# tgp-team/torch-geometric-pool

Measured on AMD Instinct MI355X. Metric: pooled nodes/sec (Reduce+Connect) on batched graphs, higher is better.
Workload: dtype f32; 1 GPU; DiffPool dense S^T X / S^T A S, batch=32 graphs N=1024 K=128 F=64 (BASELINE configs[1]); graphs_per_gpu=32, nodes_per_graph=1024, clusters=128, features=64, parallelism=graph-sharded x1

## Files before the change

### torch-geometric-pool_amd/csrc/gemm_mfma.h

```cpp
#pragma once
#include <stdlib.h>
#include <type_traits>

#include "common.h"

namespace tgp {


typedef float f32x16 __attribute__((ext_vector_type(16)));
typedef float f32x4 __attribute__((ext_vector_type(4)));

constexpr int BK = 32;
#ifndef TGP_OPERAND_PREFETCH
#define TGP_OPERAND_PREFETCH 1
#endif
#ifndef TGP_LOAD_AT
#define TGP_LOAD_AT 7
#endif
#ifndef TGP_STORE_AT
#define TGP_STORE_AT 3
#endif
#ifndef TGP_STEADY_LOOP
#define TGP_STEADY_LOOP 1
#endif
#ifndef TGP_SPREAD
#define TGP_SPREAD 1
#endif
#ifndef TGP_MIRROR_ROWS
#define TGP_MIRROR_ROWS 1
#endif
#ifndef TGP_VEC_EPILOGUE
#define TGP_VEC_EPILOGUE 1
#endif

constexpr int LDA_ROWMAJOR = BK + 1;

#ifndef TGP_SPARSE_CHUNK_GROUPS
#define TGP_SPARSE_CHUNK_GROUPS 224
#endif
#ifndef TGP_DENSE_RUN
#define TGP_DENSE_RUN 2
#endif

struct GemmRhs {
  const float* Bm;
  float* C;
  int Nc;
  long ldb, ldc, sB, sC, sCsplit;
};

struct GemmArgs {
  const float* A;
  long lda, sA;
  int M, Kd;
  GemmRhs rhs[3];
  int tiles_m, tiles_n0, tiles_n;
  int tiles_n1;
  int splits;
  int k_per_split;
  const int64_t* k_ptr;
  const int64_t* m_ptr;
  const float* resid;
  long ldr, sR;
  float* partial;
  int force_bm, force_bn;
  const int64_t* sizes;
  int accumulate;
  float* colsum;
  int colsum_skip_diag;
  int symmetric;
};

__device__ __forceinline__ int tile_row(int t) {
  const int g = t >> 3, r = t & 7;
  return 4 * (g & 7) + (r & 3) + 32 * (r >> 2) + 64 * (g >> 3);
}

#ifdef TGP_GEMM_STAMPS
__device__ unsigned long long* g_gemm_stamps = nullptr;
__device__ int g_gemm_reverse = 0;
#define TGP_STAMP(slot)                                                                        \
  do {                                                                                          \
    if (g_gemm_stamps && threadIdx.x == 0)                                                      \
      g_gemm_stamps[static_cast<long>(blockIdx.x) * 16 + (slot)] = __builtin_amdgcn_s_memrealtime(); \
  } while (0)
#else
#define TGP_STAMP(slot) do {} while (0)
#endif

__device__ __forceinline__ float4 ld4_guarded(const float* p, bool ok) {
  return ok ? *reinterpret_cast<const float4*>(p) : make_float4(0.f, 0.f, 0.f, 0.f);
}

template <bool A_KMAJOR, bool ALIGNED, int BM, int BN, int MODE, int WN = 2>
__global__ __launch_bounds__(BM * 2 * WN) void gemm_f32_mfma_kernel(GemmArgs g) {
  constexpr int THREADS = BM * 2 * WN;
  constexpr int NT = BN / (32 * WN);
  constexpr int B_TILE_FLOATS = MODE == 1 ? BN * LDA_ROWMAJOR : BK * BN;
  constexpr int BN_LANES = BN / 4;
  constexpr int A_TILE_FLOATS = BM * LDA_ROWMAJOR;
  constexpr int STAGE_FLOATS = A_TILE_FLOATS + B_TILE_FLOATS;
  constexpr int A_VECS = BM * BK / 4 / THREADS;
  constexpr int B_VECS = BN * BK / 4 / THREADS;
  constexpr int AK_LANES = BM / 4;
  constexpr bool FOLD = MODE == 4;
  constexpr bool SKIP = MODE == 3 || FOLD;
  static_assert(!FOLD || (BM == 128 && BN == 128 && WN == 4), "MODE 4: one 128 x 128 tile, 16 waves as 4 x 4");
  constexpr int NW = THREADS / 64;
  constexpr int S_ROWS = BM / NW, S_COLS = BN / 64;
  static_assert(!SKIP || (ALIGNED && S_ROWS % 2 == 0 && (S_COLS == 1 || S_COLS == 2) && NW <= 16 && BM * BN <= 2 * STAGE_FLOATS),
                "MODE 3: aligned tiles, two rows per ballot, one or two columns per lane");
  constexpr int LDA_KM = SKIP ? BM + 4 : BM;
  static_assert(BK * LDA_KM <= A_TILE_FLOATS, "k-major A tile exceeds its LDS slot");
  extern __shared__ __attribute__((aligned(16))) float smem[];
  const int tid = threadIdx.x, lane = tid & 63, wave = tid >> 6;
  const int wm = wave / WN, wn = wave % WN;
  TGP_STAMP(0);
#ifdef TGP_GEMM_STAMPS
  if (g_gemm_stamps && threadIdx.x == 0) {
    unsigned hw, xcc;
    asm volatile("s_getreg_b32 %0, hwreg(HW_REG_HW_ID)" : "=s"(hw));
    asm volatile("s_getreg_b32 %0, hwreg(HW_REG_XCC_ID)" : "=s"(xcc));
    g_gemm_stamps[static_cast<long>(blockIdx.x) * 16 + 4] = hw;
    g_gemm_stamps[static_cast<long>(blockIdx.x) * 16 + 5] = xcc;
  }
#endif

  int bid = xcd_remap(blockIdx.x, gridDim.x);
#ifdef TGP_GEMM_STAMPS
  if (g_gemm_reverse) bid = gridDim.x - 1 - bid;
#endif
  const int tn_all = bid % g.tiles_n; bid /= g.tiles_n;
  const int tm = bid % g.tiles_m; bid /= g.tiles_m;
  const int split = bid % g.splits;
  const int batch = bid / g.splits;
  const int which = tn_all >= g.tiles_n0 ? ((g.tiles_n1 && tn_all >= g.tiles_n1) ? 2 : 1) : 0;
  const int tn = which == 2 ? tn_all - g.tiles_n1 : (which ? tn_all - g.tiles_n0 : tn_all);
  const GemmRhs& R = g.rhs[which];

  const float* __restrict__ A = g.A + static_cast<long>(batch) * g.sA;
  const float* __restrict__ Bm = R.Bm + static_cast<long>(batch) * R.sB;
  float* __restrict__ C = R.C + static_cast<long>(batch) * R.sC + static_cast<long>(split) * R.sCsplit;
  const int Nc = R.Nc;
  const long lda = g.lda, ldb = R.ldb;

  const int m0 = tm * BM, n0 = tn * BN;
  if constexpr (MODE == 1) {
    if (g.sizes) {
      const int64_t nb = g.sizes[batch];
      if (m0 >= nb || n0 >= nb) {
        if (threadIdx.x == 0)
          g.partial[static_cast<long>(batch) * (g.tiles_m * g.tiles_n) + tm * g.tiles_n + tn_all] = 0.f;
        return;
      }
    }
    if (g.symmetric && m0 > n0) {
      if (threadIdx.x == 0)
        g.partial[static_cast<long>(batch) * (g.tiles_m * g.tiles_n) + tm * g.tiles_n + tn_all] = 0.f;
      return;
    }
  }
  int M = g.M;
  if (g.m_ptr) {
    const long m_lo = g.m_ptr[batch];
    M = static_cast<int>(g.m_ptr[batch + 1] - m_lo);
    if (m0 >= M) return;
    A += m_lo * lda;
    C += m_lo * R.ldc;
  }
  int k_lo = 0, k_hi = g.Kd;
  if (g.k_ptr) {
    k_lo = static_cast<int>(g.k_ptr[batch]);
    k_hi = static_cast<int>(g.k_ptr[batch + 1]);
  }
  const int k_begin = k_lo + split * g.k_per_split;
  const int k_end = min(k_hi, k_begin + g.k_per_split);
  const int nk = k_end > k_begin ? (k_end - k_begin + BK - 1) / BK : 0;

  float4 ra[2][A_VECS], rb[2][B_VECS];

  constexpr int OOB = static_cast<int>(0x80000000u);
  [[maybe_unused]] __amdgpu_buffer_rsrc_t rsrc_a, rsrc_b;
  [[maybe_unused]] int voff_a[A_VECS], voff_b[B_VECS];
  [[maybe_unused]] int kloc_a[A_VECS], kloc_b[B_VECS];
  if constexpr (ALIGNED) {
    const int a_bytes = A_KMAJOR ? (static_cast<int>(g.Kd - 1) * static_cast<int>(lda) + M) * 4
                                 : (static_cast<int>(M - 1) * static_cast<int>(lda) + g.Kd) * 4;
    const int b_bytes = MODE == 1 ? (static_cast<int>(Nc - 1) * static_cast<int>(ldb) + g.Kd) * 4
                                  : (static_cast<int>(g.Kd - 1) * static_cast<int>(ldb) + Nc) * 4;
    rsrc_a = __builtin_amdgcn_make_buffer_rsrc(const_cast<float*>(A), 0, a_bytes, 0x00020000);
    rsrc_b = __builtin_amdgcn_make_buffer_rsrc(const_cast<float*>(Bm), 0, b_bytes, 0x00020000);
#pragma unroll
    for (int i = 0; i < A_VECS; ++i) {
      if constexpr (!A_KMAJOR) {
        const int m = m0 + tile_row((tid >> 3) + i * (THREADS / 8));
        kloc_a[i] = (tid & 7) * 4;
        voff_a[i] = m < M ? (m * static_cast<int>(lda) + kloc_a[i]) * 4 : OOB;
      } else {
        const int m = m0 + (tid % AK_LANES) * 4;
        kloc_a[i] = tid / AK_LANES + i * (THREADS / AK_LANES);
        voff_a[i] = m < M ? (kloc_a[i] * static_cast<int>(lda) + m) * 4 : OOB;
      }
    }
#pragma unroll
    for (int i = 0; i < B_VECS; ++i) {
      if constexpr (MODE == 1) {
        const int n = n0 + tile_row((tid >> 3) + i * (THREADS / 8));
        kloc_b[i] = (tid & 7) * 4;
        voff_b[i] = n < Nc ? (n * static_cast<int>(ldb) + kloc_b[i]) * 4 : OOB;
      } else {
        const int n = n0 + (tid % BN_LANES) * 4;
        kloc_b[i] = tid / BN_LANES + i * (THREADS / BN_LANES);
        voff_b[i] = n < Nc ? (kloc_b[i] * static_cast<int>(ldb) + n) * 4 : OOB;
      }
    }
  }
  auto buf_ld4 = [&](__amdgpu_buffer_rsrc_t r, int voff, int soff) {
    typedef unsigned int u32x4 __attribute__((ext_vector_type(4)));
    const u32x4 v = __builtin_amdgcn_raw_buffer_load_b128(r, voff, soff, 0);
    return make_float4(__uint_as_float(v.x), __uint_as_float(v.y), __uint_as_float(v.z), __uint_as_float(v.w));
  };

  auto load_a = [&](int i, int k0, bool tail) -> float4 {
    if constexpr (ALIGNED) {
      const int soff = A_KMAJOR ? k0 * static_cast<int>(lda) * 4 : k0 * 4;
      if (!tail) return buf_ld4(rsrc_a, voff_a[i], soff);
      float4 v = buf_ld4(rsrc_a, k0 + kloc_a[i] < k_end ? voff_a[i] : OOB, soff);
      if constexpr (!A_KMAJOR) {
        const int rem = k_end - (k0 + kloc_a[i]);
        if (rem < 4) { v.w = 0.f; if (rem < 3) v.z = 0.f; if (rem < 2) v.y = 0.f; }
      }
      return v;
    } else {
      int m, k;
      if constexpr (!A_KMAJOR) {
        m = m0 + tile_row((tid >> 3) + i * (THREADS / 8));
        k = k0 + (tid & 7) * 4;
      } else {
        k = k0 + tid / AK_LANES + i * (THREADS / AK_LANES);
        m = m0 + (tid % AK_LANES) * 4;
      }
      const float* p = A_KMAJOR ? A + static_cast<long>(k) * lda + m : A + static_cast<long>(m) * lda + k;
      float t[4];
#pragma unroll
      for (int j = 0; j < 4; ++j) {
        const bool ok = A_KMAJOR ? (k < k_end && m + j < M) : (m < M && k + j < k_end);
        t[j] = ok ? p[j] : 0.f;
      }
      return make_float4(t[0], t[1], t[2], t[3]);
    }
  };
  auto load_b = [&](int i, int k0, bool tail) -> float4 {
    if constexpr (ALIGNED) {
      const int soff = MODE == 1 ? k0 * 4 : k0 * static_cast<int>(ldb) * 4;
      if (!tail) return buf_ld4(rsrc_b, voff_b[i], soff);
      float4 v = buf_ld4(rsrc_b, k0 + kloc_b[i] < k_end ? voff_b[i] : OOB, soff);
      if constexpr (MODE == 1) {
        const int rem = k_end - (k0 + kloc_b[i]);
        if (rem < 4) { v.w = 0.f; if (rem < 3) v.z = 0.f; if (rem < 2) v.y = 0.f; }
      }
      return v;
    } else {
      float t[4];
      if constexpr (MODE == 1) {
        const int n = n0 + tile_row((tid >> 3) + i * (THREADS / 8)), k = k0 + (tid & 7) * 4;
        const float* p = Bm + static_cast<long>(n) * ldb + k;
#pragma unroll
        for (int j = 0; j < 4; ++j) t[j] = (n < Nc && k + j < k_end) ? p[j] : 0.f;
      } else {
        const int k = k0 + tid / BN_LANES + i * (THREADS / BN_LANES), n = n0 + (tid % BN_LANES) * 4;
        const float* p = Bm + static_cast<long>(k) * ldb + n;
#pragma unroll
        for (int j = 0; j < 4; ++j) t[j] = (k < k_end && n + j < Nc) ? p[j] : 0.f;
      }
      return make_float4(t[0], t[1], t[2], t[3]);
    }
  };
  auto store_a = [&](int i, const float4& v, float* As) {
    if constexpr (!A_KMAJOR) {
      float* d = As + tile_row((tid >> 3) + i * (THREADS / 8)) * LDA_ROWMAJOR + (tid & 7) * 4;
      d[0] = v.x; d[1] = v.y; d[2] = v.z; d[3] = v.w;
    } else {
      *reinterpret_cast<float4*>(As + (tid / AK_LANES + i * (THREADS / AK_LANES)) * LDA_KM + (tid % AK_LANES) * 4) = v;
    }
  };
  auto store_b = [&](int i, const float4& v, float* Bs) {
    if constexpr (MODE == 1) {
      float* d = Bs + tile_row((tid >> 3) + i * (THREADS / 8)) * LDA_ROWMAJOR + (tid & 7) * 4;
      d[0] = v.x; d[1] = v.y; d[2] = v.z; d[3] = v.w;
    } else {
      *reinterpret_cast<float4*>(Bs + (tid / BN_LANES + i * (THREADS / BN_LANES)) * BN + (tid % BN_LANES) * 4) = v;
    }
  };

  f32x16 acc[NT];
#pragma unroll
  for (int j = 0; j < NT; ++j)
#pragma unroll
    for (int r = 0; r < 16; ++r) acc[j][r] = 0.f;

  const int lm = lane & 31, lk = lane >> 5;
  float rres[MODE == 1 ? NT : 1][16];
  [[maybe_unused]] float rmir[MODE == 1 ? NT : 1][16];
  [[maybe_unused]] const bool mirror = MODE == 1 && g.symmetric && m0 < n0;
  constexpr bool MIRROR_PATCH_FITS = (THREADS / 64) * (32 * 33) <= 2 * STAGE_FLOATS;
  [[maybe_unused]] const bool mirror_rows = mirror && MIRROR_PATCH_FITS && TGP_MIRROR_ROWS && (g.ldr & 3) == 0 &&
                                            (reinterpret_cast<uintptr_t>(g.resid + static_cast<long>(batch) * g.sR) & 15) == 0 &&
                                            m0 + BM <= M && n0 + BN <= Nc && n0 + BN <= M && m0 + BM <= Nc;
  if constexpr (MODE == 1) {
    const float* __restrict__ Rm = g.resid + static_cast<long>(batch) * g.sR;
#pragma unroll
    for (int j = 0; j < NT; ++j) {
      const int col = n0 + wn * (BN / WN) + j * 32 + lm;
#pragma unroll
      for (int r = 0; r < 16; ++r) {
        const int row = m0 + wm * 32 + (r & 3) + 8 * (r >> 2) + 4 * lk;
        rres[j][r] = (row < M && col < Nc) ? Rm[static_cast<long>(row) * g.ldr + col] : 0.f;
      }
    }
    if (mirror && mirror_rows) {
      const float* __restrict__ base = Rm + static_cast<long>(n0 + wn * (BN / WN) + (lane >> 3)) * g.ldr + m0 + wm * 32 +
                                       4 * (lane & 7);
#pragma unroll
      for (int j = 0; j < NT; ++j)
#pragma unroll
        for (int q = 0; q < 4; ++q) {
          const float4 v = *reinterpret_cast<const float4*>(base + static_cast<long>(j * 32 + 8 * q) * g.ldr);
          rmir[j][4 * q] = v.x; rmir[j][4 * q + 1] = v.y; rmir[j][4 * q + 2] = v.z; rmir[j][4 * q + 3] = v.w;
        }
    } else if (mirror) {
      const bool v4 = (g.ldr & 3) == 0 && (reinterpret_cast<uintptr_t>(Rm) & 15) == 0;
#pragma unroll
      for (int j = 0; j < NT; ++j) {
        const int col = n0 + wn * (BN / WN) + j * 32 + lm;
#pragma unroll
        for (int q = 0; q < 4; ++q) {
          const int row = m0 + wm * 32 + 8 * q + 4 * lk;
          const float* src = Rm + static_cast<long>(col) * g.ldr + row;
          if (v4 && col < Nc && row + 3 < M) {
            const float4 v = *reinterpret_cast<const float4*>(src);
            rmir[j][4 * q] = v.x; rmir[j][4 * q + 1] = v.y; rmir[j][4 * q + 2] = v.z; rmir[j][4 * q + 3] = v.w;
          } else {
#pragma unroll
            for (int u = 0; u < 4; ++u) rmir[j][4 * q + u] = (col < Nc && row + u < M) ? src[u] : 0.f;
          }
        }
      }
    }
  }
  const int a_off = A_KMAJOR ? lk * LDA_KM + wm * 32 + lm : (wm * 32 + lm) * LDA_ROWMAJOR + lk;
  const int a_step = A_KMAJOR ? 2 * LDA_KM : 2;
  const int b_off = MODE == 1 ? (wn * (BN / WN) + lm) * LDA_ROWMAJOR + lk : lk * BN + wn * (BN / WN) + lm;
  constexpr int b_step = MODE == 1 ? 2 : 2 * BN;
  constexpr int b_tile = MODE == 1 ? 32 * LDA_ROWMAJOR : 32;
  constexpr int PD = TGP_OPERAND_PREFETCH;
  float a_r[PD + 1], b_r[PD + 1][NT];
  auto fetch_pair = [&](const float* As, const float* Bs, int p) {
    a_r[p % (PD + 1)] = As[a_off + p * a_step];
#pragma unroll
    for (int j = 0; j < NT; ++j) b_r[p % (PD + 1)][j] = Bs[b_off + p * b_step + b_tile * j];
  };
  auto mfma_pair = [&](int p) {
#pragma unroll
    for (int j = 0; j < NT; ++j)
      acc[j] = __builtin_amdgcn_mfma_f32_32x32x2f32(a_r[p % (PD + 1)], b_r[p % (PD + 1)][j], acc[j], 0, 0, 0);
  };

  [[maybe_unused]] unsigned* chunk_rec = reinterpret_cast<unsigned*>(smem + 2 * STAGE_FLOATS);
  [[maybe_unused]] float sacc[SKIP ? S_ROWS : 1][S_COLS];
  [[maybe_unused]] bool any_sparse = false;
  if constexpr (SKIP) {
#pragma unroll
    for (int j = 0; j < S_ROWS; ++j)
#pragma unroll
      for (int c = 0; c < S_COLS; ++c) sacc[j][c] = 0.f;
  }
  auto record_chunk = [&](auto par, const auto& va, const auto& vb) {
    unsigned n = 0;
#pragma unroll
    for (int i = 0; i < A_VECS; ++i)
      n += __popcll(__ballot(((__float_as_uint(va[i].x) | __float_as_uint(va[i].y) | __float_as_uint(va[i].z) |
                               __float_as_uint(va[i].w)) << 1) != 0u));
    unsigned mag = 0;
#pragma unroll
    for (int i = 0; i < B_VECS; ++i)
      mag = max(max(mag, max(__float_as_uint(vb[i].x) & 0x7fffffffu, __float_as_uint(vb[i].y) & 0x7fffffffu)),
                max(__float_as_uint(vb[i].z) & 0x7fffffffu, __float_as_uint(vb[i].w) & 0x7fffffffu));
    if (__ballot(mag >= 0x7f800000u)) n += 1u << 16;
    if (lane == 0) chunk_rec[par * 16 + wave] = n;
  };
  auto chunk_is_sparse = [&](auto par) -> bool {
    const uint4* r = reinterpret_cast<const uint4*>(chunk_rec + par * 16);
    unsigned n = 0;
#pragma unroll
    for (int q = 0; q < NW / 4; ++q) {
      const uint4 v = r[q];
      n += v.x + v.y + v.z + v.w;
    }
    return __builtin_amdgcn_readfirstlane(n) <= TGP_SPARSE_CHUNK_GROUPS;
  };
  auto sparse_chunk = [&](auto As, auto Bs) {
    float va[S_ROWS / 2];
#pragma unroll
    for (int i = 0; i < S_ROWS / 2; ++i) {
      const int row = wave + NW * (2 * i + (lane >> 5)), k = lane & 31;
      va[i] = A_KMAJOR ? As[k * LDA_KM + row] : As[row * LDA_ROWMAJOR + k];
    }
#pragma unroll
    for (int i = 0; i < S_ROWS / 2; ++i) asm volatile("" : "+v"(va[i]));
#pragma unroll
    for (int i = 0; i < S_ROWS / 2; ++i) {
      const float v = va[i];
      const unsigned long long nz = __ballot(v != 0.f);
      const int vbits = __float_as_int(v);
#pragma unroll
      for (int h = 0; h < 2; ++h) {
        for (unsigned m = static_cast<unsigned>(nz >> (32 * h)); m; m &= m - 1) {
          const int kk = __builtin_ctz(m);
          const float a = __int_as_float(__builtin_amdgcn_readlane(vbits, kk + 32 * h));
          if constexpr (S_COLS == 2) {
            const float2 b = *reinterpret_cast<const float2*>(Bs + kk * BN + 2 * lane);
            sacc[2 * i + h][0] = fmaf(a, b.x, sacc[2 * i + h][0]);
            sacc[2 * i + h][S_COLS - 1] = fmaf(a, b.y, sacc[2 * i + h][S_COLS - 1]);
          } else {
            sacc[2 * i + h][0] = fmaf(a, Bs[kk * BN + lane], sacc[2 * i + h][0]);
          }
        }
      }
    }
  };

  float* L0 = smem;
  float* L1 = smem + STAGE_FLOATS;
  auto kof = [&](int t) { return k_begin + t * BK; };
  [[maybe_unused]] int dense_run = 0;
  [[maybe_unused]] bool dense_rest = false;
  auto stage = [&](auto par_c, auto steady_c, auto sk_c, int t) {
    constexpr int PAR = decltype(par_c)::value;
    constexpr bool STEADY = decltype(steady_c)::value;
    constexpr bool SK = decltype(sk_c)::value;
    const float* As = PAR ? L1 : L0;
    const float* Bs = As + A_TILE_FLOATS;
    float* An = PAR ? L0 : L1;
    float* Bn = An + A_TILE_FLOATS;
    const bool do_store = STEADY || t + 1 < nk, do_load = STEADY || t + 2 < nk;
    const int k2 = kof(t + 2);
    const bool tail = !STEADY && k2 + BK > k_end;
#ifdef TGP_GEMM_STAMPS
    const bool probe = g_gemm_stamps && t == (nk / 2) && threadIdx.x == 0;
#define TGP_PHASE(i) do { if (probe) g_gemm_stamps[static_cast<long>(blockIdx.x) * 16 + 8 + (i)] = __builtin_amdgcn_s_memrealtime(); } while (0)
#else
#define TGP_PHASE(i) do {} while (0)
#endif
    TGP_PHASE(0);
    bool sparse = false;
    if constexpr (SK) {
#pragma unroll
      for (int p = 0; p < PD; ++p) fetch_pair(As, Bs, p);
      sparse = chunk_is_sparse(PAR);
#pragma unroll
      for (int p = 0; p < PD; ++p) {
        asm volatile("" ::"v"(a_r[p % (PD + 1)]));
#pragma unroll
        for (int j = 0; j < NT; ++j) asm volatile("" ::"v"(b_r[p % (PD + 1)][j]));
      }
      any_sparse = any_sparse || sparse;
      dense_run = sparse ? 0 : dense_run + 1;
      dense_rest = dense_run >= TGP_DENSE_RUN;
      if (sparse) {
#pragma unroll
      for (int v = 0; v < A_VECS + B_VECS; ++v)
        if (do_load) {
          if (v < A_VECS) ra[PAR][v] = load_a(v, k2, tail);
          else rb[PAR][v - A_VECS] = load_b(v - A_VECS, k2, tail);
        }
      sparse_chunk(As, Bs);
#pragma unroll
      for (int v = 0; v < A_VECS + B_VECS; ++v)
        if (do_store) {
          if (v < A_VECS) store_a(v, ra[1 - PAR][v], An);
          else store_b(v - A_VECS, rb[1 - PAR][v - A_VECS], Bn);
        }
      if (do_store) record_chunk(1 - PAR, ra[1 - PAR], rb[1 - PAR]);
#pragma unroll
      for (int j = 0; j < NT; ++j) asm volatile("" : "+v"(acc[j]));
      }
    }
    if (!SK || !sparse) {
    if constexpr (!SK) {
#pragma unroll
      for (int p = 0; p < PD; ++p) fetch_pair(As, Bs, p);
    }
#pragma unroll
    for (int p = 0; p < BK / 2; ++p) {
      if (p + PD < BK / 2) fetch_pair(As, Bs, p + PD);
      mfma_pair(p);
      if (p + PD < BK / 2) __builtin_amdgcn_sched_group_barrier(0x100, 1 + NT, 0);
      __builtin_amdgcn_sched_group_barrier(0x008, NT, 0);
      constexpr int LOAD_AT = TGP_LOAD_AT, STORE_AT = TGP_STORE_AT, SPREAD = TGP_SPREAD;
      if (p == STORE_AT) TGP_PHASE(1);
      if (p == LOAD_AT) TGP_PHASE(3);
#pragma unroll
      for (int v = 0; v < A_VECS + B_VECS; ++v) {
        if (p == LOAD_AT + (SPREAD ? v : 0) && do_load) {
          if (v < A_VECS) ra[PAR][v] = load_a(v, k2, tail);
          else rb[PAR][v - A_VECS] = load_b(v - A_VECS, k2, tail);
        }
        if (p == STORE_AT + (SPREAD ? v : 0) && do_store) {
          if (v < A_VECS) store_a(v, ra[1 - PAR][v], An);
          else store_b(v - A_VECS, rb[1 - PAR][v - A_VECS], Bn);
        }
      }
      if constexpr (SK) {
        if (p == STORE_AT + (SPREAD ? A_VECS + B_VECS : 1) && do_store) record_chunk(1 - PAR, ra[1 - PAR], rb[1 - PAR]);
      }
      __builtin_amdgcn_sched_barrier(0);
      if (p == STORE_AT) TGP_PHASE(2);
      if (p == LOAD_AT) TGP_PHASE(4);
    }
    }
    TGP_PHASE(5);
    __syncthreads();
    TGP_PHASE(6);
  };
  if (nk > 0) {
#pragma unroll
    for (int i = 0; i < A_VECS; ++i) ra[0][i] = load_a(i, kof(0), kof(0) + BK > k_end);
#pragma unroll
    for (int i = 0; i < B_VECS; ++i) rb[0][i] = load_b(i, kof(0), kof(0) + BK > k_end);
  }
  if (nk > 1) {
#pragma unroll
    for (int i = 0; i < A_VECS; ++i) ra[1][i] = load_a(i, kof(1), kof(1) + BK > k_end);
#pragma unroll
    for (int i = 0; i < B_VECS; ++i) rb[1][i] = load_b(i, kof(1), kof(1) + BK > k_end);
  }
  if (nk > 0) {
#pragma unroll
    for (int i = 0; i < A_VECS; ++i) store_a(i, ra[0][i], L0);
#pragma unroll
    for (int i = 0; i < B_VECS; ++i) store_b(i, rb[0][i], L0 + A_TILE_FLOATS);
    if constexpr (SKIP) record_chunk(0, ra[0], rb[0]);
  }
  __syncthreads();
  TGP_STAMP(1);
  [[maybe_unused]] float4 fs[4], fx[2];
  auto fold_load = [&]() {
    if constexpr (FOLD) {
      const GemmRhs& RX = g.rhs[1];
      const int x_bytes = RX.Bm ? static_cast<int>(g.Kd) * static_cast<int>(RX.ldb) * 4 : 0;
      const __amdgpu_buffer_rsrc_t rsrc_x = __builtin_amdgcn_make_buffer_rsrc(
          const_cast<float*>(RX.Bm ? RX.Bm + static_cast<long>(batch) * RX.sB : Bm), 0, x_bytes, 0x00020000);
      const int ldx4 = RX.Bm ? static_cast<int>(RX.ldb) * 4 : 0;
      const int voff_x = (RX.Bm && (tid & 15) * 4 < RX.Nc) ? (tid >> 4) * ldx4 + (tid & 15) * 16 : OOB;
#pragma unroll
      for (int i = 0; i < 4; ++i) fs[i] = buf_ld4(rsrc_b, voff_b[0], (m0 + 32 * i) * static_cast<int>(ldb) * 4);
#pragma unroll
      for (int i = 0; i < 2; ++i) fx[i] = buf_ld4(rsrc_x, voff_x, (m0 + 64 * i) * ldx4);
    }
  };
  int t = 0;
  using std::integral_constant;
  using FALSE_C = integral_constant<bool, false>;
  using TRUE_C = integral_constant<bool, true>;
  if constexpr (!SKIP) {
  if constexpr (ALIGNED && TGP_STEADY_LOOP) {
    for (; t + 3 < nk && kof(t + 3) + BK <= k_end; t += 2) {
#ifdef TGP_GEMM_STAMPS
      if (t == (nk / 2 & ~1)) TGP_STAMP(6);
      if (t == ((3 * nk) / 4 & ~1)) TGP_STAMP(7);
#endif
      stage(integral_constant<int, 0>{}, TRUE_C{}, FALSE_C{}, t);
      stage(integral_constant<int, 1>{}, TRUE_C{}, FALSE_C{}, t + 1);
    }
  }
  for (; t < nk; t += 2) {
#ifdef TGP_GEMM_STAMPS
    if (t == (nk / 2 & ~1)) TGP_STAMP(6);
    if (t == ((3 * nk) / 4 & ~1)) TGP_STAMP(7);
#endif
    stage(integral_constant<int, 0>{}, FALSE_C{}, FALSE_C{}, t);
    if (t + 1 < nk) stage(integral_constant<int, 1>{}, FALSE_C{}, FALSE_C{}, t + 1);
  }
  } else {
    for (; t + 3 < nk && kof(t + 3) + BK <= k_end && !dense_rest; t += 2) {
      stage(integral_constant<int, 0>{}, TRUE_C{}, TRUE_C{}, t);
      stage(integral_constant<int, 1>{}, TRUE_C{}, TRUE_C{}, t + 1);
    }
    for (; t + 3 < nk && kof(t + 3) + BK <= k_end; t += 2) {
      stage(integral_constant<int, 0>{}, TRUE_C{}, FALSE_C{}, t);
      stage(integral_constant<int, 1>{}, TRUE_C{}, FALSE_C{}, t + 1);
    }
    auto tail_stage = [&](auto par_c, int t) {
      if (dense_rest) stage(par_c, FALSE_C{}, FALSE_C{}, t);
      else stage(par_c, FALSE_C{}, TRUE_C{}, t);
    };
    for (; t < nk; t += 2) {
      tail_stage(integral_constant<int, 0>{}, t);
      if (t + 1 < nk) tail_stage(integral_constant<int, 1>{}, t + 1);
    }
  }
  TGP_STAMP(2);
  fold_load();
  if constexpr (SKIP && !FOLD) {
    if (any_sparse) {
#pragma unroll
      for (int j = 0; j < S_ROWS; ++j)
#pragma unroll
        for (int c = 0; c < S_COLS; ++c) smem[(wave + NW * j) * BN + S_COLS * lane + c] = sacc[j][c];
      __syncthreads();
#pragma unroll
      for (int j = 0; j < NT; ++j)
#pragma unroll
        for (int r = 0; r < 16; ++r)
          acc[j][r] = __fadd_rn(acc[j][r],
                                smem[(wm * 32 + (r & 3) + 8 * (r >> 2) + 4 * lk) * BN + wn * (BN / WN) + j * 32 + lm]);
      __syncthreads();
    }
  }

  if constexpr (FOLD) {
    constexpr int P_LD = 196;
    float* Sf = smem;
    float* UXf = smem + BM * BN;
    const GemmRhs& RX = g.rhs[1];
    const int F = RX.Bm ? RX.Nc : 0;
    const int l15 = lane & 15, lq = lane >> 4;
#pragma unroll
    for (int i = 0; i < 4; ++i) {
      const int k = (tid >> 5) + 32 * i;
      *reinterpret_cast<float4*>(Sf + k * BN + (((tid & 31) * 4) ^ ((k & 3) << 4))) = fs[i];
    }
#pragma unroll
    for (int i = 0; i < 2; ++i) {
      const int k = (tid >> 4) + 64 * i;
      *reinterpret_cast<float4*>(UXf + k * 192 + ((BN + (tid & 15) * 4) ^ ((k & 3) << 4))) = fx[i];
    }
#pragma unroll
    for (int r = 0; r < 16; ++r) {
      const int rl = (r & 3) + 8 * (r >> 2) + 4 * lk;
      UXf[(wm * 32 + rl) * 192 + ((wn * 32 + lm) ^ ((r & 3) << 4))] = m0 + wm * 32 + rl < M ? acc[0][r] : 0.f;
    }
    f32x4 d[2][3];
#pragma unroll
    for (int i = 0; i < 2; ++i)
#pragma unroll
      for (int j = 0; j < 3; ++j)
#pragma unroll
        for (int r = 0; r < 4; ++r) d[i][j][r] = 0.f;
    __syncthreads();
    if (any_sparse) {
#pragma unroll
      for (int j = 0; j < S_ROWS; ++j) {
        const int row = wave + NW * j;
        float2* u = reinterpret_cast<float2*>(UXf + row * 192 + ((2 * lane) ^ ((row & 3) << 4)));
        float2 v = *u;
        v.x = __fadd_rn(v.x, sacc[j][0]);
        v.y = __fadd_rn(v.y, sacc[j][S_COLS - 1]);
        *u = v;
      }
      __syncthreads();
    }
    TGP_STAMP(8);
    {
      int a_at[2], b_at[3];
#pragma unroll
      for (int i = 0; i < 2; ++i) a_at[i] = lq * BN + ((wm * 32 + 16 * i + l15) ^ (lq << 4));
#pragma unroll
      for (int j = 0; j < 3; ++j) b_at[j] = lq * 192 + ((wn * 48 + 16 * j + l15) ^ (lq << 4));
      float a[2][2], b[2][3];
      auto fetch = [&](int s) {
#pragma unroll
        for (int i = 0; i < 2; ++i) a[s & 1][i] = Sf[4 * s * BN + a_at[i]];
#pragma unroll
        for (int j = 0; j < 3; ++j) b[s & 1][j] = UXf[4 * s * 192 + b_at[j]];
      };
      fetch(0);
#pragma unroll
      for (int s = 0; s < 32; ++s) {
        if (s + 1 < 32) fetch(s + 1);
#pragma unroll
        for (int j = 0; j < 3; ++j)
#pragma unroll
          for (int i = 0; i < 2; ++i)
            d[i][j] = __builtin_amdgcn_mfma_f32_16x16x4f32(a[s & 1][i], b[s & 1][j], d[i][j], 0, 0, 0);
        if (s + 1 < 32) __builtin_amdgcn_sched_group_barrier(0x100, 5, 0);
        __builtin_amdgcn_sched_group_barrier(0x008, 6, 0);
        __builtin_amdgcn_sched_barrier(0);
      }
    }
    TGP_STAMP(9);
    __syncthreads();
    bool used[3];
#pragma unroll
    for (int j = 0; j < 3; ++j) {
      const int c0 = wn * 48 + 16 * j;
      used[j] = c0 < BN ? c0 < Nc : c0 - BN < F;
    }
    float* P = smem;
#pragma unroll
    for (int i = 0; i < 2; ++i)
#pragma unroll
      for (int j = 0; j < 3; ++j)
        if (used[j]) {
#pragma unroll
          for (int r = 0; r < 4; ++r) P[(wm * 32 + 16 * i + 4 * lq + r) * P_LD + wn * 48 + 16 * j + l15] = d[i][j][r];
        }
    __syncthreads();
    TGP_STAMP(10);
    if (g.colsum) {
      float* part = smem + BM * P_LD;
      const int j = tid & (BN - 1), q = tid >> 7;
      float cs = 0.f;
#pragma unroll
      for (int u = 0; u < 16; ++u) {
        const int row = 16 * q + u;
        const float v = P[row * P_LD + j];
        cs = __fadd_rn(cs, (row >= Nc || (g.colsum_skip_diag && row == j)) ? 0.f : v);
      }
      part[q * BN + j] = cs;
      __syncthreads();
      if (tid < Nc) {
        float tot = 0.f;
#pragma unroll
        for (int qq = 0; qq < 8; ++qq) tot = __fadd_rn(tot, part[qq * BN + tid]);
        g.colsum[(static_cast<long>(batch) * g.tiles_m + tm) * Nc + tid] = tot;
      }
    }
    TGP_STAMP(11);
    float* Ca = R.C + static_cast<long>(batch) * R.sC + static_cast<long>(tm) * R.sCsplit;
    const int kq = Nc >> 2, fq = F >> 2;
    for (int e = tid; e < Nc * kq; e += THREADS) {
      const int row = e / kq, c4 = (e - row * kq) * 4;
      *reinterpret_cast<float4*>(Ca + static_cast<long>(row) * R.ldc + c4) = *reinterpret_cast<const float4*>(P + row * P_LD + c4);
    }
    if (F) {
      float* Cx = RX.C + static_cast<long>(batch) * RX.sC + static_cast<long>(tm) * RX.sCsplit;
      for (int e = tid; e < Nc * fq; e += THREADS) {
        const int row = e / fq, c4 = (e - row * fq) * 4;
        *reinterpret_cast<float4*>(Cx + static_cast<long>(row) * RX.ldc + c4) =
            *reinterpret_cast<const float4*>(P + row * P_LD + BN + c4);
      }
    }
    TGP_STAMP(3);
    return;
  }

  if constexpr (MODE == 1) {
    float sq = 0.f;
#pragma unroll
    for (int j = 0; j < NT; ++j)
#pragma unroll
      for (int r = 0; r < 16; ++r) {
        const float d = rres[j][r] - acc[j][r];
        sq = fmaf(d, d, sq);
      }
    if (mirror && mirror_rows) {
      float* patch = smem + wave * (32 * 33);
#pragma unroll
      for (int j = 0; j < NT; ++j) {
#pragma unroll
        for (int q = 0; q < 4; ++q) {
          float* d = patch + ((lane >> 3) + 8 * q) * 33 + 4 * (lane & 7);
          d[0] = rmir[j][4 * q]; d[1] = rmir[j][4 * q + 1]; d[2] = rmir[j][4 * q + 2]; d[3] = rmir[j][4 * q + 3];
        }
        __builtin_amdgcn_wave_barrier();
#pragma unroll
        for (int r = 0; r < 16; ++r) {
          const float d = patch[lm * 33 + (r & 3) + 8 * (r >> 2) + 4 * lk] - acc[j][r];
          sq = fmaf(d, d, sq);
        }
        __builtin_amdgcn_wave_barrier();
      }
    } else if (mirror) {
#pragma unroll
      for (int j = 0; j < NT; ++j)
#pragma unroll
        for (int r = 0; r < 16; ++r) {
          const float d = rmir[j][r] - acc[j][r];
          sq = fmaf(d, d, sq);
        }
    }
#pragma unroll
    for (int o = 32; o > 0; o >>= 1) sq += __shfl_xor(sq, o, 64);
    __syncthreads();
    if (lane == 0) smem[wave] = sq;
    __syncthreads();
    if (tid == 0) {
      float t = 0.f;
      for (int w = 0; w < THREADS / 64; ++w) t += smem[w];
      g.partial[static_cast<long>(batch) * (g.tiles_m * g.tiles_n) + tm * g.tiles_n + tn_all] = t;
    }
    return;
  }
  constexpr bool PATCH_FITS = (THREADS / 64) * (32 * 36) <= 2 * STAGE_FLOATS;
  const bool vec_store = ALIGNED && PATCH_FITS && TGP_VEC_EPILOGUE && !g.accumulate && (R.ldc & 3) == 0 &&
                         (reinterpret_cast<uintptr_t>(C) & 15) == 0 && m0 + BM <= M && n0 + BN <= Nc;
  if (vec_store) {
    float* patch = smem + wave * (32 * 36);
#pragma unroll
    for (int j = 0; j < NT; ++j) {
#pragma unroll
      for (int r = 0; r < 16; ++r) patch[((r & 3) + 8 * (r >> 2) + 4 * lk) * 36 + lm] = acc[j][r];
      __builtin_amdgcn_wave_barrier();
      const int c4 = (lane & 7) * 4, r8 = lane >> 3;
#pragma unroll
      for (int q = 0; q < 4; ++q) {
        const int rr = r8 + 8 * q;
        const float4 v = *reinterpret_cast<const float4*>(patch + rr * 36 + c4);
        *reinterpret_cast<float4*>(C + static_cast<long>(m0 + wm * 32 + rr) * R.ldc + n0 + wn * (BN / WN) + j * 32 + c4) = v;
      }
      __builtin_amdgcn_wave_barrier();
    }
  } else {
#pragma unroll
  for (int j = 0; j < NT; ++j) {
    const int col = n0 + wn * (BN / WN) + j * 32 + lm;
#pragma unroll
    for (int r = 0; r < 16; ++r) {
      const int row = m0 + wm * 32 + (r & 3) + 8 * (r >> 2) + 4 * lk;
      if (row < M && col < Nc) {
        float* dst = C + static_cast<long>(row) * R.ldc + col;
        *dst = g.accumulate ? __fadd_rn(*dst, acc[j][r]) : acc[j][r];
      }
    }
  }
  }
  if constexpr (MODE == 2) {
    if (vec_store) __syncthreads();
    if (g.colsum && which == 0) {
      if (m0 + BM > M) {
        const int rows_left = M - (m0 + wm * 32 + 4 * lk);
#pragma unroll
        for (int j = 0; j < NT; ++j)
#pragma unroll
          for (int r = 0; r < 16; ++r)
            if ((r & 3) + 8 * (r >> 2) >= rows_left) acc[j][r] = 0.f;
      }
#pragma unroll
      for (int j = 0; j < NT; ++j) {
        float cs = 0.f;
        const int dcol = n0 + wn * (BN / WN) + j * 32 + lm - (m0 + wm * 32 + 4 * lk);
#pragma unroll
        for (int r = 0; r < 16; ++r)
          cs = __fadd_rn(cs, (g.colsum_skip_diag && (r & 3) + 8 * (r >> 2) == dcol) ? 0.f : acc[j][r]);
        cs = wave_fold<64, 32>(cs, op_fadd_rn{});
        if (lk == 0) smem[wm * BN + wn * (BN / WN) + j * 32 + lm] = cs;
      }
      __syncthreads();
      if (tid < BN && n0 + tid < Nc) {
        float tot = 0.f;
#pragma unroll
        for (int q = 0; q < BM / 32; ++q) tot = __fadd_rn(tot, smem[q * BN + tid]);
        g.colsum[((static_cast<long>(batch) * g.splits + split) * g.tiles_m + tm) * Nc + n0 + tid] = tot;
      }
    }
  }
  TGP_STAMP(3);
}

static bool gemm_aligned(const GemmArgs& g, bool ) {
  static const bool force_scalar = getenv("TGP_GEMM_SCALAR") && atoi(getenv("TGP_GEMM_SCALAR"));
  if (force_scalar) return false;
  auto ok = [](const void* p, long, long) { return reinterpret_cast<uintptr_t>(p) % 4 == 0; };
  bool a = ok(g.A, g.lda, g.sA);
  const long lim = (1l << 31) - 4096;
  a = a && (static_cast<long>(g.M) * g.lda * 4 < lim) && (static_cast<long>(g.Kd) * g.lda * 4 < lim);
  for (int w = 0; w < 3; ++w)
    if (w == 0 || (w == 1 && g.tiles_n > g.tiles_n0) || (w == 2 && g.tiles_n1))
      a = a && ok(g.rhs[w].Bm, g.rhs[w].ldb, g.rhs[w].sB) &&
          (static_cast<long>(g.Kd) * g.rhs[w].ldb * 4 < lim) && (static_cast<long>(g.rhs[w].Nc) * g.rhs[w].ldb * 4 < lim);
  return a;
}

struct TileCfg { int bm, bn; };
static TileCfg pick_tile(int64_t M, int64_t max_nc, int64_t batches_x_splits, const GemmArgs& g) {
  static const int fbm = getenv("TGP_GEMM_BM") ? atoi(getenv("TGP_GEMM_BM")) : 0;
  static const int fbn = getenv("TGP_GEMM_BN") ? atoi(getenv("TGP_GEMM_BN")) : 0;
  TileCfg t{128, 128};
  auto count = [&](int bm, int bn) {
    int64_t tn = 0;
    tn += (g.rhs[0].Nc + bn - 1) / bn;
    if (g.rhs[1].Bm) tn += (g.rhs[1].Nc + bn - 1) / bn;
    if (g.rhs[1].Bm && g.rhs[2].Bm) tn += (g.rhs[2].Nc + bn - 1) / bn;
    return ((M + bm - 1) / bm) * tn * batches_x_splits;
  };
  if (M <= 64) t.bm = 64;
  if (count(t.bm, 128) < 2 * 256 && max_nc >= 64) t.bn = 64;
  if (count(t.bm, t.bn) < 2 * 256 && t.bm == 128 && M > 64) t.bm = 64;
  if (g.force_bm) t.bm = g.force_bm;
  if (g.force_bn) t.bn = g.force_bn;
  if (fbm == 64 || fbm == 128) t.bm = fbm;
  if (fbn == 64 || fbn == 128) t.bn = fbn;
  return t;
}

template <bool A_KMAJOR, int BM, int BN, int MODE = 0, int WN = 2>
static void launch_gemm_cfg(const GemmArgs& g_in, int batches, hipStream_t stream) {
  const GemmArgs& g = g_in;
  const int nwg = batches * g.splits * g.tiles_m * g.tiles_n;
  const size_t lds = 2 * (BM * LDA_ROWMAJOR + (MODE == 1 ? BN * LDA_ROWMAJOR : BK * BN)) * sizeof(float);
  if (gemm_aligned(g, A_KMAJOR && MODE == 0))
    hipLaunchKernelGGL((gemm_f32_mfma_kernel<A_KMAJOR, true, BM, BN, MODE, WN>), dim3(nwg), dim3(BM * 2 * WN), lds, stream, g);
  else
    hipLaunchKernelGGL((gemm_f32_mfma_kernel<A_KMAJOR, false, BM, BN, MODE, WN>), dim3(nwg), dim3(BM * 2 * WN), lds, stream, g);
}

template <bool A_KMAJOR>
static bool launch_gemm(GemmArgs g, int batches, hipStream_t stream, int* tiles_m_out = nullptr) {
  int64_t max_nc = g.rhs[1].Bm && g.rhs[1].Nc > g.rhs[0].Nc ? g.rhs[1].Nc : g.rhs[0].Nc;
  const bool third = g.rhs[1].Bm && g.rhs[2].Bm;
  if (third && g.rhs[2].Nc > max_nc) max_nc = g.rhs[2].Nc;
  const TileCfg t = pick_tile(g.M, max_nc, static_cast<int64_t>(batches) * g.splits, g);
  g.tiles_m = cdiv(g.M, t.bm);
  g.tiles_n0 = cdiv(g.rhs[0].Nc, t.bn);
  g.tiles_n = g.tiles_n0 + (g.rhs[1].Bm ? cdiv(g.rhs[1].Nc, t.bn) : 0);
  g.tiles_n1 = 0;
  if (third) {
    g.tiles_n1 = g.tiles_n;
    g.tiles_n += cdiv(g.rhs[2].Nc, t.bn);
  }
  if (tiles_m_out) *tiles_m_out = g.tiles_m;
  if (t.bm == 64 && t.bn == 64 && g.colsum) {
    launch_gemm_cfg<A_KMAJOR, 64, 64, 2>(g, batches, stream);
    return true;
  }
  if (t.bm == 64 && t.bn == 64) launch_gemm_cfg<A_KMAJOR, 64, 64>(g, batches, stream);
  else if (t.bm == 64) launch_gemm_cfg<A_KMAJOR, 64, 128>(g, batches, stream);
  else if (t.bn == 64) launch_gemm_cfg<A_KMAJOR, 128, 64>(g, batches, stream);
  else launch_gemm_cfg<A_KMAJOR, 128, 128, 0, 4>(g, batches, stream);
  return false;
}

template <bool A_KMAJOR>
static void launch_gemm_skip_zeros(GemmArgs g, int batches, hipStream_t stream) {
  if (g.splits != 1 || g.accumulate || g.rhs[1].Bm || g.colsum || g.m_ptr || g.k_ptr || !gemm_aligned(g, A_KMAJOR)) {
    launch_gemm<A_KMAJOR>(g, batches, stream);
    return;
  }
  constexpr int BM = 128, BN = 128, WN = 4;
  const int tiles_m = cdiv(g.M, BM), tiles_n = cdiv(g.rhs[0].Nc, BN);
  const int nwg = batches * tiles_m * tiles_n;
  if (nwg < 256) {
    launch_gemm<A_KMAJOR>(g, batches, stream);
    return;
  }
  g.tiles_m = tiles_m;
  g.tiles_n0 = g.tiles_n = tiles_n;
  g.tiles_n1 = 0;
  const size_t lds = 2 * (BM * LDA_ROWMAJOR + BK * BN) * sizeof(float) + 2 * 16 * sizeof(unsigned);
  hipLaunchKernelGGL((gemm_f32_mfma_kernel<A_KMAJOR, true, BM, BN, 3, WN>), dim3(nwg), dim3(BM * 2 * WN), lds, stream, g);
}

constexpr int FOLD_BM = 128, FOLD_MAX_F = 64;
static int fold_tiles(int64_t N, int64_t K, int64_t F) {
  return (K <= 128 && K % 4 == 0 && F <= FOLD_MAX_F && F % 4 == 0) ? cdiv(N, FOLD_BM) : 0;
}
template <bool A_KMAJOR>
static bool launch_gemm_fold(GemmArgs g, int batches, hipStream_t stream) {
  constexpr int BM = FOLD_BM, BN = 128, WN = 4;
  const GemmRhs x = g.rhs[1];
  g.rhs[1] = GemmRhs{};
  const long lim = (1l << 31) - 4096;
  if (!gemm_aligned(g, A_KMAJOR) || g.rhs[0].Nc > BN ||
      (x.Bm && (reinterpret_cast<uintptr_t>(x.Bm) % 4 != 0 || x.Nc > FOLD_MAX_F || (static_cast<long>(g.Kd) + BM) * x.ldb * 4 >= lim)))
    return false;
  g.rhs[1] = x;
  g.tiles_m = cdiv(g.M, BM);
  g.tiles_n0 = g.tiles_n = 1;
  g.tiles_n1 = 0;
  g.splits = 1;
  const int nwg = batches * g.tiles_m;
  if (nwg < 256) return false;
  constexpr size_t lds = (BM * BN + BM * 192) * sizeof(float);
  static_assert(BM * BN + BM * 192 >= BM * 196 + 8 * BN && BM * 196 + 8 * BN >= 2 * (BM * LDA_ROWMAJOR + BK * BN) + 2 * 16,
                "MODE 4: the tail's operands cover its result tile, which covers the k-loop's stages");
  (void)hipFuncSetAttribute(reinterpret_cast<const void*>(gemm_f32_mfma_kernel<A_KMAJOR, true, BM, BN, 4, WN>),
                            hipFuncAttributeMaxDynamicSharedMemorySize, static_cast<int>(lds));
  hipLaunchKernelGGL((gemm_f32_mfma_kernel<A_KMAJOR, true, BM, BN, 4, WN>), dim3(nwg), dim3(BM * 2 * WN), lds, stream, g);
  return true;
}

static int launch_gemm_residual(GemmArgs g, int batches, hipStream_t stream, bool dry_run = false) {
  TileCfg t = pick_tile(g.M, g.rhs[0].Nc, batches, g);
  if (g.symmetric && g.Kd <= 8 * BK && !g.force_bm && !g.force_bn && t.bm == 128 && t.bn == 128) t = TileCfg{64, 64};
  g.tiles_m = cdiv(g.M, t.bm);
  g.tiles_n0 = g.tiles_n = cdiv(g.rhs[0].Nc, t.bn);
  if (dry_run) return g.tiles_m * g.tiles_n;
  static const int no_sym = getenv("TGP_LINK_LOSS_FULL") ? atoi(getenv("TGP_LINK_LOSS_FULL")) : 0;
  if (t.bm != t.bn || g.M != g.rhs[0].Nc || g.rhs[0].Bm != g.A || g.rhs[0].sB != g.sA || g.rhs[0].ldb != g.lda || no_sym)
    g.symmetric = 0;
  if (t.bm == 64 && t.bn == 64) launch_gemm_cfg<false, 64, 64, 1>(g, batches, stream);
  else if (t.bm == 64) launch_gemm_cfg<false, 64, 128, 1>(g, batches, stream);
  else if (t.bn == 64) launch_gemm_cfg<false, 128, 64, 1>(g, batches, stream);
  else launch_gemm_cfg<false, 128, 128, 1, 4>(g, batches, stream);
  return g.tiles_m * g.tiles_n;
}

}
```

Before: 504.7 million nodes/s.

## Add wide-K sparse front-end that walks nonzeros before the dense MFMA loop

Adds a front-end stage to the skip-zeros GEMM kernel (row-major A, 128x128 tiles). It loads 128-wide K chunks of A and B, counts nonzero groups per wave, and while a chunk is sparse enough it accumulates only the nonzero A entries into sacc using scalar FMAs. It then hands the remaining K range to the existing MFMA pipeline. The aim is to skip multiply work on very sparse adjacency chunks. In exchange it needs a larger LDS allocation, which may lower occupancy, and it adds ballot/transpose overhead when chunks turn out dense.

Result: faster. 546.8 million nodes/s (median of 6 runs) (+8.3%).

```diff
diff --git a/torch-geometric-pool_amd/csrc/gemm_mfma.h b/torch-geometric-pool_amd/csrc/gemm_mfma.h
--- a/torch-geometric-pool_amd/csrc/gemm_mfma.h
+++ b/torch-geometric-pool_amd/csrc/gemm_mfma.h
@@ -37,6 +37,9 @@
 
 #ifndef TGP_SPARSE_CHUNK_GROUPS
 #define TGP_SPARSE_CHUNK_GROUPS 224
+#endif
+#ifndef TGP_SPARSE_WIDE_GROUPS
+#define TGP_SPARSE_WIDE_GROUPS 896
 #endif
 #ifndef TGP_DENSE_RUN
 #define TGP_DENSE_RUN 2
@@ -173,9 +176,9 @@
     k_lo = static_cast<int>(g.k_ptr[batch]);
     k_hi = static_cast<int>(g.k_ptr[batch + 1]);
   }
-  const int k_begin = k_lo + split * g.k_per_split;
+  int k_begin = k_lo + split * g.k_per_split;
   const int k_end = min(k_hi, k_begin + g.k_per_split);
-  const int nk = k_end > k_begin ? (k_end - k_begin + BK - 1) / BK : 0;
+  int nk = k_end > k_begin ? (k_end - k_begin + BK - 1) / BK : 0;
 
   float4 ra[2][A_VECS], rb[2][B_VECS];
 
@@ -523,6 +526,106 @@
     __syncthreads();
     TGP_PHASE(6);
   };
+  constexpr bool FRONT = SKIP && !A_KMAJOR && BM == 128 && BN == 128 && WN == 4;
+  if constexpr (FRONT) {
+    constexpr int WIDE_K = 128;
+    constexpr int W_FLOATS = WIDE_K * BN;
+    constexpr int W_VECS = WIDE_K * BN / 4 / THREADS;
+    constexpr int W_PAIRS = S_ROWS / 2;
+    constexpr int W_REGS = S_ROWS * (WIDE_K / 64);
+    typedef unsigned int u32x4 __attribute__((ext_vector_type(4)));
+    unsigned* wide_rec = reinterpret_cast<unsigned*>(smem + 2 * W_FLOATS);
+    unsigned* wide_turn = wide_rec + 2 * 16 + wave * 256;
+    u32x4 wr[W_PAIRS];
+    unsigned wa[W_REGS];
+    float4 ws[W_VECS];
+    int voff_w[W_PAIRS];
+#pragma unroll
+    for (int i = 0; i < W_PAIRS; ++i) {
+      const int m = m0 + wave + NW * (2 * i + (lane >> 5));
+      voff_w[i] = m < M ? (m * static_cast<int>(lda) + 4 * (lane & 31)) * 4 : OOB;
+    }
+    auto wide_load = [&](int k0) {
+#pragma unroll
+      for (int i = 0; i < W_PAIRS; ++i) wr[i] = __builtin_amdgcn_raw_buffer_load_b128(rsrc_a, voff_w[i], k0 * 4, 0);
+#pragma unroll
+      for (int i = 0; i < W_VECS; ++i)
+        ws[i] = buf_ld4(rsrc_b, voff_b[0], (k0 + i * (THREADS / BN_LANES)) * static_cast<int>(ldb) * 4);
+    };
+    auto wide_publish = [&](auto par_c) {
+      constexpr int PAR = decltype(par_c)::value;
+#pragma unroll
+      for (int i = 0; i < W_VECS; ++i) store_b(i, ws[i], smem + PAR * W_FLOATS);
+      unsigned n = 0;
+#pragma unroll
+      for (int i = 0; i < W_PAIRS; ++i) {
+        n += __popcll(__ballot(((wr[i].x | wr[i].y | wr[i].z | wr[i].w) << 1) != 0u));
+        *reinterpret_cast<u32x4*>(wide_turn + 4 * lane) = wr[i];
+        __builtin_amdgcn_wave_barrier();
+#pragma unroll
+        for (int q = 0; q < 4; ++q) wa[4 * i + q] = wide_turn[64 * q + lane];
+        __builtin_amdgcn_wave_barrier();
+      }
+      unsigned mag = 0;
+#pragma unroll
+      for (int i = 0; i < W_VECS; ++i)
+        mag = max(max(mag, max(__float_as_uint(ws[i].x) & 0x7fffffffu, __float_as_uint(ws[i].y) & 0x7fffffffu)),
+                  max(__float_as_uint(ws[i].z) & 0x7fffffffu, __float_as_uint(ws[i].w) & 0x7fffffffu));
+      if (__ballot(mag >= 0x7f800000u)) n += 1u << 16;
+      if (lane == 0) wide_rec[PAR * 16 + wave] = n;
+    };
+    auto wide_is_sparse = [&](auto par_c) -> bool {
+      const uint4* r = reinterpret_cast<const uint4*>(wide_rec + decltype(par_c)::value * 16);
+      unsigned n = 0;
+#pragma unroll
+      for (int q = 0; q < NW / 4; ++q) {
+        const uint4 v = r[q];
+        n += v.x + v.y + v.z + v.w;
+      }
+      return __builtin_amdgcn_readfirstlane(n) <= TGP_SPARSE_WIDE_GROUPS;
+    };
+    auto wide_walk = [&](auto par_c) {
+      const float* Bs = smem + decltype(par_c)::value * W_FLOATS;
+#pragma unroll
+      for (int r = 0; r < W_REGS; ++r) {
+        constexpr int PARTS = WIDE_K / 64;
+        const int j = r / PARTS;
+        const float* Bp = Bs + 64 * (r % PARTS) * BN + 2 * lane;
+        const int vbits = static_cast<int>(wa[r]);
+        for (unsigned long long m = __ballot(__int_as_float(vbits) != 0.f); m; m &= m - 1) {
+          const int kk = __builtin_ctzll(m);
+          const float a = __int_as_float(__builtin_amdgcn_readlane(vbits, kk));
+          const float2 b = *reinterpret_cast<const float2*>(Bp + kk * BN);
+          sacc[j][0] = fmaf(a, b.x, sacc[j][0]);
+          sacc[j][1] = fmaf(a, b.y, sacc[j][1]);
+        }
+      }
+    };
+    int kw = k_begin;
+    if (k_end - kw >= WIDE_K) {
+      using P0 = std::integral_constant<int, 0>;
+      using P1 = std::integral_constant<int, 1>;
+      wide_load(kw);
+      wide_publish(P0{});
+      __syncthreads();
+      auto wide_stage = [&](auto par_c) -> bool {
+        constexpr int PAR = decltype(par_c)::value;
+        if (!wide_is_sparse(par_c)) return false;
+        const bool more = k_end - kw >= 2 * WIDE_K;
+        if (more) wide_load(kw + WIDE_K);
+        wide_walk(par_c);
+        if (more) wide_publish(std::integral_constant<int, 1 - PAR>{});
+        any_sparse = true;
+        kw += WIDE_K;
+        __syncthreads();
+        return more;
+      };
+      while (wide_stage(P0{}) && wide_stage(P1{})) {
+      }
+      k_begin = kw;
+      nk = k_end > k_begin ? (k_end - k_begin + BK - 1) / BK : 0;
+    }
+  }
   if (nk > 0) {
 #pragma unroll
     for (int i = 0; i < A_VECS; ++i) ra[0][i] = load_a(i, kof(0), kof(0) + BK > k_end);
@@ -948,7 +1051,12 @@
   g.tiles_m = tiles_m;
   g.tiles_n0 = g.tiles_n = tiles_n;
   g.tiles_n1 = 0;
-  const size_t lds = 2 * (BM * LDA_ROWMAJOR + BK * BN) * sizeof(float) + 2 * 16 * sizeof(unsigned);
+  constexpr size_t lds = A_KMAJOR ? 2 * (BM * LDA_ROWMAJOR + BK * BN) * sizeof(float) + 2 * 16 * sizeof(unsigned)
+                                  : 2 * 128 * BN * sizeof(float) + (2 * 16 + 16 * 256) * sizeof(unsigned);
+  static_assert(A_KMAJOR || 2 * 128 * BN >= 2 * (BM * LDA_ROWMAJOR + BK * BN) + 2 * 16, "MODE 3: the wide chunks cover the stages");
+  if constexpr (!A_KMAJOR)
+    (void)hipFuncSetAttribute(reinterpret_cast<const void*>(gemm_f32_mfma_kernel<A_KMAJOR, true, BM, BN, 3, WN>),
+                              hipFuncAttributeMaxDynamicSharedMemorySize, static_cast<int>(lds));
   hipLaunchKernelGGL((gemm_f32_mfma_kernel<A_KMAJOR, true, BM, BN, 3, WN>), dim3(nwg), dim3(BM * 2 * WN), lds, stream, g);
 }
 
@@ -975,6 +1083,7 @@
   constexpr size_t lds = (BM * BN + BM * 192) * sizeof(float);
   static_assert(BM * BN + BM * 192 >= BM * 196 + 8 * BN && BM * 196 + 8 * BN >= 2 * (BM * LDA_ROWMAJOR + BK * BN) + 2 * 16,
                 "MODE 4: the tail's operands cover its result tile, which covers the k-loop's stages");
+  static_assert(BM * BN + BM * 192 >= 2 * 128 * BN + 2 * 16 + 16 * 256, "MODE 4: ... and the wide front-end's two Bm chunks, records and turn areas");
   (void)hipFuncSetAttribute(reinterpret_cast<const void*>(gemm_f32_mfma_kernel<A_KMAJOR, true, BM, BN, 4, WN>),
                             hipFuncAttributeMaxDynamicSharedMemorySize, static_cast<int>(lds));
   hipLaunchKernelGGL((gemm_f32_mfma_kernel<A_KMAJOR, true, BM, BN, 4, WN>), dim3(nwg), dim3(BM * 2 * WN), lds, stream, g);
```
